# AnteMarusic/Accelerating-Genomics

Hardware: AMD Instinct MI355X
Metric: Smith-Waterman affine-gap score-only GCUPS (config 2: 65536 pairs 150x150 per GPU) (higher is better)
Workload: dtype int16x2 lanes, int32 scores; 1 GPU; BASELINE config 2: 65536 SW pairs 150x150 per GPU, iid ACGT + 25% related, newline sentinel aligned as the reference does; pairs_per_gpu=65536, len=150, cells_counted_per_pair=22500, parallelism=pairs sharded per GPU, no collective

## Files before the change

accelerating-genomics_amd/api.py:

```python
from __future__ import annotations

import ctypes as C
import os
import subprocess

import numpy as np

_HERE = os.path.dirname(os.path.abspath(__file__))
TUNING_KNOBS = ("AGX_SW_KERNEL", "AGX_SW_TAIL_BETA", "AGX_SW_MAX_C", "AGX_SW_FORCE_C", "AGX_SW_MAX_CLASSES", "AGX_SW_WAVES_PER_CLASS",
                "AGX_SW_SORT_WAVES", "AGX_SW_ONE_LAUNCH", "AGX_SW_DNA", "AGX_SW_RISE", "AGX_SW_PERIOD", "AGX_PHMM_PLAIN_CELL", "AGX_TRACE_CREATE", "AGX_HOST_THREADS", "AGX_FANOUT", "AGX_PHMM_TAB_BUDGET", "AGX_PHMM_MAX_C",
                "AGX_PHMM_FORCE_C", "AGX_PHMM_TAIL_BETA", "AGX_PHMM_MAX_CLASSES", "AGX_PHMM_NO_LUT", "AGX_TRACE_POOL", "AGX_NO_STREAM_PRIO", "AGX_SW_I32_CLASSIC", "AGX_SW_PIECE_MB", "AGX_SW_PIECE_MIN_PAIRS", "AGX_PHMM_NO_ROWS", "AGX_PHMM_NO_TRAINS", "AGX_PHMM_LUT_ONE_LOOP", "AGX_SW_HOST_PLAN", "AGX_PHMM_NO_RING", "AGX_TRACE_CIGAR")
_DEFAULT_LIB = "libagx_tuning.so" if any(k in os.environ for k in TUNING_KNOBS) else "libagx.so"
LIB_PATH = os.environ.get("AGX_LIB_PATH", os.path.join(_HERE, _DEFAULT_LIB))

OK, E_ARG, E_NODEVICE, E_HIP, E_NOMEM, E_SYMBOL, E_LIMIT, E_IO, E_INTERNAL = 0, -1, -2, -3, -4, -5, -6, -7, -8
SW_ALIGN_ENDS, SW_ALIGN_SPANS = 1, 2
SW_ALIGN_MAX_QUERY_LEN, SW_ALIGN_MAX_TARGET_LEN = 2560, 65535
SW_MODE_LOCAL, SW_MODE_GLOBAL, SW_MODE_FIT, SW_MODE_EXTEND, SW_MODE_EXTEND_QUERY = 0, 1, 2, 3, 4
SwHit = np.dtype([("score", np.int32), ("a_begin", np.int32), ("a_end", np.int32), ("b_begin", np.int32), ("b_end", np.int32)])
SwStat = np.dtype([("matches", np.int32), ("pairs", np.int32)])
SW_STATS_MAX_QUERY_LEN = 1792
SW_CIGAR_MAX_QUERY_LEN = 2048
SW_BAND_MAX_LEN = 65535
SW_BAND_MAX_WIDTH = 2048
CIGAR_INS, CIGAR_DEL, CIGAR_EQ, CIGAR_DIFF = 1, 2, 7, 8
_CIGAR_CHARS = {CIGAR_INS: "I", CIGAR_DEL: "D", CIGAR_EQ: "=", CIGAR_DIFF: "X"}
OPT_SW_KERNEL = 1
OPT_SW_PLANNER = 2
SW_PLANNER_AUTO, SW_PLANNER_HOST, SW_PLANNER_DEVICE = 0, 1, 2
OPT_PHMM_TRAINS = 3
OPT_SW_TRACE_BYTES = 4
PHMM_TRAINS_AUTO, PHMM_TRAINS_OFF, PHMM_TRAINS_ON = 0, 1, 2
SW_KERNEL_AUTO, SW_KERNEL_INT32, SW_KERNEL_PACKED_SIGNED, SW_KERNEL_PACKED_BIASED = 0, 1, 2, 3
PHMM_F64, PHMM_F64_FMA, PHMM_F32, PHMM_F32_FMA = 0, 1, 2, 3
# ... 663 lines not shown
```

accelerating-genomics_amd/csrc/agx_sw.cpp:

```cpp
#include "agx_sw_batch.h"

#include <cmath>
#include <memory>
#include <mutex>
#include <thread>

#include "agx_parallel.h"

using namespace agx_sw_host;

namespace {

struct Tiling {
    int cls;
    int G;
};

bool positive(long n) { return n > 0; }
bool at_least_4(long n) { return n >= 4; }
inline double tail_beta_override() { static const double v = agx_knob_real(agx_tune("AGX_SW_TAIL_BETA"), -1.0); return v; }
int max_cols_per_lane() { static const int v = (int)agx_knob_int(agx_tune("AGX_SW_MAX_C"), AGX_SW_MAX_COLS_PER_LANE, at_least_4); return v; }
int force_cols_per_lane() { static const int v = (int)agx_knob_int(agx_tune("AGX_SW_FORCE_C"), 0); return v; }
int max_classes_override() { static const int v = (int)agx_knob_int(agx_tune("AGX_SW_MAX_CLASSES"), 0, positive); return v; }
int tuned_kernel()
// ... 121 lines not shown
    return best;
}

inline uint64_t piece_bytes() { static const uint64_t v = (uint64_t)agx_knob_int(agx_tune("AGX_SW_PIECE_MB"), 32, positive) << 20; return v; }
inline int64_t piece_min_pairs() { static const int64_t v = agx_knob_int(agx_tune("AGX_SW_PIECE_MIN_PAIRS"), 32768, positive); return v; }
constexpr size_t kRawPad = 64;
constexpr uint8_t kClsEmpty = 255;
constexpr uint8_t kClsUntiled = 254;
struct PairPlan {
    uint32_t pair;
    uint32_t ly;
    uint16_t lxo;
    uint8_t cls;
    uint8_t G;
    uint32_t lx() const { return lxo & 0x7fffu; }
};

struct Bucket {
    size_t first = 0, count = 0;
    size_t group0 = 0, n_groups = 0;
    size_t wave0 = 0, n_waves = 0;
    int cls = 0, G = 0;
};

}

namespace {
int finish_create(agx_sw_batch *b);
void drop_pending(agx_sw_batch *b);
}

extern "C" {

void agx_sw_batch_destroy(agx_sw_batch *b)
{
    if (!b) return;
    if (b->ctx) (void)hipSetDevice(b->ctx->device);
    drop_pending(b);
    b->img.release();
    b->groups.release();
    b->waves.release();
    b->scores.release();
    b->table.release();
    b->out_stage.release();
    b->ends.release();
    b->ends_stage.release();
// ... 815 lines not shown
    t_sort = agx_now_ms();
    }

    size_t n_groups = 0, n_waves_total = 0, groups_bytes = 0, waves_bytes = 0;
    const size_t img0 = packed ? (size_t)kSwPackedMaxShort / 4 + 1 : 0;
    size_t img_dw = img0;
    std::vector<SwWave> waves;
    std::vector<ClassLaunch> launches;
    uint32_t launched_classes = 0;
    int64_t padded = 0;
    double t_waves = t_sort, t_records = t_sort;
    std::vector<uint8_t> groups_host;
    if (device_plan) {
        {
            static std::mutex once_per_context;
            std::lock_guard<std::mutex> l(once_per_context);
            rc = agx_ctx_prepare_plan(ctx);
        }
        if (!rc) rc = dp.h_buckets.alloc(ctx, (size_t)kSwPlanBuckets * 5 * sizeof(uint32_t));
        if (rc) return rc;
        uint32_t *bt = (uint32_t *)dp.h_buckets.p;
        size_t entries = 0, n_waves = 0;
        uint32_t class_mask = 0;
        for (int k = 0; k < kSwPlanBuckets; ++k) {
            const size_t count = dp.hist[(size_t)k];
            const int G = 64 - (k & 63);
            const size_t ng = (count + slots - 1) / slots, per_wave = (size_t)(64 / G), nw = (ng + per_wave - 1) / per_wave;
            bt[5 * k + 0] = (uint32_t)entries;
            bt[5 * k + 1] = (uint32_t)count;
            bt[5 * k + 2] = (uint32_t)n_groups;
            bt[5 * k + 3] = (uint32_t)ng;
            bt[5 * k + 4] = (uint32_t)n_waves;
            entries += count;
            n_groups += ng;
            n_waves += nw;
            if (count) class_mask |= 1u << (k >> 6);
        }
        n_waves_total = n_waves;
        launched_classes = class_mask;
        img_dw = dp.img_dw;
        groups_bytes = n_groups * sizeof(SwGroup2);
        waves_bytes = n_waves * sizeof(SwWave);
        ClassLaunch cl;
        cl.C = (class_mask & (class_mask - 1)) ? 0 : kSwClasses[__builtin_ctz(class_mask)];
        cl.first_wave = 0;
        cl.n_waves = (uint32_t)n_waves;
        launches.assign(1, cl);
        rc = launch_device_plan(ctx, dp, b, (uint32_t)n_pairs, (uint32_t)entries, longest_long, slots, (uint32_t)img0, n_groups, n_waves);
        if (!rc) rc = h_flag.alloc(ctx, 2 * sizeof(uint32_t));
        if (rc) return rc;
        t_waves = t_records = agx_now_ms();
    } else {
    std::vector<Bucket> bk;
    for (size_t i = 0; i < plan.size();) {
        Bucket q;
        q.first = i;
        q.cls = plan[i].cls;
        q.G = plan[i].G;
        size_t lo = i, hi = plan.size();
        while (lo + 1 < hi) {
            const size_t mid = lo + (hi - lo) / 2;
            if (plan[mid].cls == q.cls && plan[mid].G == q.G) lo = mid;
            else hi = mid;
        }
        q.count = lo + 1 - i;
        i = lo + 1;
        bk.push_back(q);
    }
    size_t n_waves = 0;
// ... 32 lines not shown
        const char *e = agx_tune("AGX_SW_SORT_WAVES");
        return !(e && e[0] == '0');
    }();
    static const bool one_launch_ok = [] {
        const char *e = agx_tune("AGX_SW_ONE_LAUNCH");
        return !(e && e[0] == '0');
    }();
    if (coded_plan && launches.size() > 1 && one_launch_ok) {
        if (sort_waves)
            std::stable_sort(waves.begin(), waves.end(), [](const SwWave &a, const SwWave &b) {
                return (uint64_t)a.steps * a.reserved > (uint64_t)b.steps * b.reserved;
            });
        ClassLaunch all_classes;
        all_classes.C = 0;
        all_classes.first_wave = 0;
        all_classes.n_waves = (uint32_t)waves.size();
        launches.assign(1, all_classes);
    } else if (sort_waves && !launches.empty())
        agx_pool_run((int)launches.size(), [&](int k) {
            const ClassLaunch &cl = launches[(size_t)k];
            std::stable_sort(waves.begin() + cl.first_wave, waves.begin() + cl.first_wave + cl.n_waves,
                             [](const SwWave &a, const SwWave &b) { return a.steps > b.steps; });
        });
    std::vector<uint32_t> x_dw(plan.size()), y_dw(plan.size());
    img_dw = img0;
    {
        const int parts = (int)std::min<int64_t>(agx_host_threads(), std::max<int64_t>(1, (int64_t)plan.size() / 16384));
        std::vector<size_t> part_sum((size_t)parts + 1, 0);
        const size_t chunk = (plan.size() + parts - 1) / (size_t)parts;
        auto words = [&](const PairPlan &pp, size_t *xw) {
            *xw = ((size_t)pp.G * kSwClasses[pp.cls] + 3) / 4 + 1;
            return *xw + ((size_t)pp.ly + 3) / 4;
        };
        agx_pool_run(parts, [&](int t) {
            const size_t lo = std::min(plan.size(), (size_t)t * chunk), hi = std::min(plan.size(), lo + chunk);
            size_t s = 0, xw;
            for (size_t i = lo; i < hi; ++i) s += words(plan[i], &xw);
            part_sum[(size_t)t + 1] = s;
        });
        for (int t = 0; t < parts; ++t) part_sum[(size_t)t + 1] += part_sum[(size_t)t];
        img_dw = img0 + part_sum[(size_t)parts];
        if (img_dw > 0xffffffffull) {
            agx_set_error("packed image exceeds 16 GiB; split the batch");
            return AGX_E_LIMIT;
        }
        agx_pool_run(parts, [&](int t) {
// ... 217 lines not shown
        return AGX_E_NODEVICE;
    }
    int rc = agx_bind(b->ctx);
    if (rc) return rc;
    if (b->banded) return band_launch(b);
    if (b->pending && b->pending->ready) AGX_HIP(hipStreamWaitEvent(b->ctx->stream, b->pending->ready, 0));
    SwParams prm = b->prm;
    if (b->bound) prm.n_out = (uint32_t)b->n_pairs;
    b->cig_valid = false;
    if (b->cigar == 2 && !b->trace_p && b->tr_dwords) {
        agx_set_error("agx_sw_batch_launch: a traced fill without its trace block");
        return AGX_E_INTERNAL;
    }
    FanOut fan(b->ctx, (int)b->launches.size());
    rc = fan.begin();
    if (rc) return rc;
    int k = 0;
    for (auto it = b->launches.rbegin(); it != b->launches.rend(); ++it) {
        const ClassLaunch &cl = *it;
        hipStream_t st = fan.stream(k++);
        const uint32_t *img = (const uint32_t *)b->img.p;
        const SwWave *wv = (const SwWave *)b->waves.p + cl.first_wave;
        int32_t *scores = b->bound ? b->bound : (int32_t *)b->scores.p;
        const int anch_capture = b->mode != AGX_SW_MODE_EXTEND, anch_flags = b->mode == AGX_SW_MODE_FIT ? 1 : b->mode == AGX_SW_MODE_GLOBAL ? 2 : 0;
        int r;
        uint32_t *lstat = (uint32_t *)b->lstat.p;
        if (b->cigar == 2 && b->matrix)
            r = agx_sw_trace_mat_launch_class(cl.C, prm, img, (const SwGroup *)b->groups.p, wv, cl.n_waves, scores, (uint32_t *)b->ends.p, b->trace_p,
                                              (const uint64_t *)b->goff.p, (const int16_t *)b->table.p, st);
        else if (b->cigar == 2)
            r = agx_sw_trace_launch_class(cl.C, prm, img, (const SwGroup *)b->groups.p, wv, cl.n_waves, scores, (uint32_t *)b->ends.p, b->trace_p,
                                          (const uint64_t *)b->goff.p, st);
        else if (b->stats == 2 && b->family == 5 && b->matrix)
            r = agx_sw_anch_mat_stats_launch_class(cl.C, anch_capture, anch_flags, prm, img, (const SwGroup *)b->groups.p, wv, cl.n_waves, scores,
                                                   (uint32_t *)b->ends.p, lstat, (const int16_t *)b->table.p, st);
        else if (b->stats == 2 && b->family == 5)
            r = agx_sw_anch_stats_launch_class(cl.C, anch_capture, anch_flags, prm, img, (const SwGroup *)b->groups.p, wv, cl.n_waves, scores,
                                               (uint32_t *)b->ends.p, lstat, st);
        else if (b->stats == 2 && b->matrix)
            r = agx_sw_loc_mat_stats_launch_class(cl.C, prm, img, (const SwGroup *)b->groups.p, wv, cl.n_waves, scores, (uint32_t *)b->ends.p, lstat,
                                                  (const int16_t *)b->table.p, st);
        else if (b->stats == 2)
            r = agx_sw_loc_stats_launch_class(cl.C, prm, img, (const SwGroup *)b->groups.p, wv, cl.n_waves, scores, (uint32_t *)b->ends.p, lstat, st);
        else if (b->family == 5 && b->matrix)
            r = agx_sw_anch_mat_launch_class(cl.C, anch_capture, anch_flags, prm, img, (const SwGroup *)b->groups.p, wv, cl.n_waves, scores,
                                             (uint32_t *)b->ends.p, (const int16_t *)b->table.p, st);
// ... 210 lines not shown
```

accelerating-genomics_amd/csrc/agx_sw.h:

```cpp
#pragma once
#include <hip/hip_runtime.h>

#include <algorithm>
#include <cstdint>

#include "../../include/agx.h"

struct SwGroup {
    uint32_t x_dw;
    uint32_t y_dw;
    uint32_t lx_ly;
    uint32_t out;
};

struct SwParams {
    int32_t ge;
    int32_t gf;
    int32_t hd;
    int32_t delta;
    int32_t shift;
    uint32_t ge2, gf2, hd2, delta2;
    uint32_t age2, agf2, bias2;
    uint32_t n_out;
};

struct SwGroup2 {
    uint32_t x_dw[2];
    uint32_t y_dw[2];
    uint32_t lx_ly[2];
    uint32_t out[2];
};

struct SwWave {
    uint32_t first_group;
    uint16_t n_groups;
    uint16_t G;
    uint32_t steps;
    uint32_t reserved;
};

#define AGX_SW_FOR_EACH_CLASS(X) \
    X(4) X(6) X(8) X(10) X(12) X(14) X(16) X(18) X(20) X(22) X(24) X(26) X(28) X(30) X(32) X(34) X(36) X(38) X(40)
#define AGX_SW_FOR_EACH_WIDE_CLASS(X) X(80) X(120) X(160)
static const int kSwClasses[] = {4, 6, 8, 10, 12, 14, 16, 18, 20, 22, 24, 26, 28, 30, 32, 34, 36, 38, 40, 80, 120, 160};
static const int kSwPackedMaxShort = 64 * 40;
static const int kSwNumClasses = sizeof(kSwClasses) / sizeof(kSwClasses[0]);
static const double kSwClassCost[] = {1.373, 1.250, 1.178, 1.138, 1.112, 1.080, 1.051, 1.033, 1.025, 1.022, 1.014, 1.014, 1.011, 1.007, 1.007, 1.004, 1.004, 1.004, 1.000, 1.6, 2.2, 4.0};
static const double kSwPkClassCost[] = {1.543, 1.358, 1.278, 1.210, 1.173, 1.136, 1.111, 1.086, 1.068, 1.037, 1.025, 1.025, 1.019, 1.012, 1.006, 1.006, 1.006, 1.000, 1.000, 0, 0, 0};
static const double kSwPk2ClassCost[] = {1.851, 1.581, 1.450, 1.367, 1.318, 1.263, 1.196, 1.184, 1.145, 1.097, 1.095, 1.056, 1.049, 1.053, 1.025, 1.023, 1.022, 1.016, 1.000, 0, 0, 0};

static const double kSwI32dClassCost[] = {1.373, 1.250, 1.178, 1.138, 1.112, 1.080, 1.051, 1.033, 1.025, 1.022, 1.014, 1.014, 1.011, 1.007, 1.007, 1.004, 1.004, 1.004, 1.000, 0, 0, 0};

constexpr int kSwMatDim = 33;
int agx_sw_mat_launch_class(int cols_per_lane, const SwParams &prm, const uint32_t *img, const SwGroup *groups,
                            const SwWave *waves, uint32_t n_waves, int32_t *scores, const int16_t *table, hipStream_t s);
int agx_sw_pack_launch(bool matrix, int slots, const uint8_t *raw, const uint64_t *off, uint64_t base, const void *groups,
                       uint32_t n_groups, uint32_t n_pairs, uint32_t *img, const uint8_t *code, uint32_t *flag, int n_cu,
                       hipStream_t s);
int agx_sw_pack_dna_launch(const uint8_t *raw, const uint64_t *off, uint64_t base, void *groups, void *waves, uint32_t n_waves,
                           uint32_t n_pairs, uint32_t *img, uint32_t *flag, int n_cu, hipStream_t s);
int agx_sw_pk_launch_class(int cols_per_lane, const SwParams &prm, const uint32_t *img, const SwGroup2 *groups,
                           const SwWave *waves, uint32_t n_waves, int32_t *scores, hipStream_t s);
// ... 147 lines not shown
```

accelerating-genomics_amd/csrc/agx_sw_batch.h:

```cpp
#pragma once
#include "agx_sw.h"

#include <algorithm>

#include "agx_internal.h"

namespace agx_sw_host __attribute__((visibility("hidden"))) {

struct ClassLaunch {
    int C = 0;
    uint32_t first_wave = 0, n_waves = 0;
};

}

struct agx_sw_batch {
    agx_ctx *ctx = nullptr;
    int family = 0;
    int align = 0;
    int mode = 0;
    int stats = 0;
    DevBuf lstat;
    PinBuf lstat_stage;
    int cigar = 0;
    std::vector<uint64_t> tr_goff;
    std::vector<SwWalkRec> tr_walk;
    uint64_t tr_dwords = 0, tr_slot_words = 0;
    DevBuf goff, walkrec;
    uint32_t *trace_p = nullptr;
    bool cig_valid = false;
    std::vector<agx_sw_hit> cig_hits;
    std::vector<uint64_t> cig_off;
    std::vector<uint32_t> cig_ops;
    agx_sw_cigar_info cig_info{};
// ... 87 lines not shown
```

accelerating-genomics_amd/csrc/agx_sw_pack_kernel.hip:

```cpp
#include "agx_sw.h"

namespace {

template <bool MAT>
__device__ __forceinline__ uint32_t fetch(const uint8_t *__restrict__ seq, uint32_t idx, uint32_t len,
                                          const uint8_t *__restrict__ code, bool &bad)
{
    if (idx >= len) return 0u;
    uint32_t b = seq[idx];
    if constexpr (MAT) {
        const uint32_t c = code[b];
        bad |= c == 0xffu;
        b = (c + 1u) & 0xffu;
    } else
        bad |= b == 0u;
    return b;
}

template <bool MAT>
__device__ __forceinline__ void copy_seq(uint32_t *__restrict__ dst, uint32_t n_dw, const uint8_t *__restrict__ seq, uint32_t len,
                                         const uint8_t *__restrict__ code, int lane, bool &bad)
{
    for (uint32_t i = lane; i < n_dw; i += 64) {
        uint32_t v = 0;
// ... 75 lines not shown

__device__ __forceinline__ uint32_t find_entry(const uint32_t *s_pre, uint32_t c)
{
    uint32_t lo = 0;
#pragma unroll
    for (uint32_t step = kPackEntries / 2; step; step >>= 1)
        if (s_pre[lo + step] <= c) lo += step;
    return lo;
}

__global__ void __launch_bounds__(256) sw_pack_dna(const uint8_t *__restrict__ raw, const uint64_t *__restrict__ off, uint64_t base,
                                                   uint32_t *__restrict__ groups, uint32_t *__restrict__ waves, uint32_t n_fill_waves,
                                                   uint32_t n_pairs, uint32_t *__restrict__ img, uint32_t *__restrict__ flag)
{
    __shared__ uint32_t s_bits[128][8];
    __shared__ uint64_t s_src[kPackEntries];
    __shared__ uint32_t s_len[kPackEntries];
    __shared__ uint32_t s_flags[kPackEntries];
    __shared__ uint32_t s_pre[kPackEntries + 1];
    __shared__ uint32_t s_wsum[4];
    __shared__ uint32_t s_info[128], s_syms[128];
    __shared__ uint32_t s_dst[kPackEntries], s_wlen[kPackEntries];
    __shared__ uint32_t s_not_dna;
    const uint32_t e = threadIdx.x, sl = e >> 1, which = e & 1u;
    for (uint32_t i = threadIdx.x; i < 128 * 8; i += 256) (&s_bits[0][0])[i] = 0;
    for (uint32_t fw = blockIdx.x; fw < n_fill_waves; fw += gridDim.x) {
        const uint32_t first_group = waves[4 * (size_t)fw], n_groups = waves[4 * (size_t)fw + 1] & 0xffffu;
        const uint32_t gc = (waves[4 * (size_t)fw + 1] >> 16) * (waves[4 * (size_t)fw + 3] & 0xffffu);
        const uint32_t n_slots = n_groups * 2u;
        if (threadIdx.x == 0) s_not_dna = 0;
        uint32_t *rec = groups + (size_t)(first_group + (sl >> 1)) * 8u;
        const uint32_t h = sl & 1u;
        uint32_t len = 0, nl = 0, x_dw = 0, y_dw = 0, lx = 0, ly = 0, xsec = 0, out = n_pairs;
        uint64_t src = 0;
        if (sl < n_slots) {
            x_dw = rec[h], y_dw = rec[2 + h];
            const uint32_t ll = rec[4 + h];
            out = rec[6 + h];
            if (out < n_pairs) {
                lx = ll & 0x7fffu, xsec = (ll >> 15) & 1u, ly = ll >> 16;
                src = off[2 * (size_t)out + (which ? xsec ^ 1u : xsec)] - base;
                len = which ? ly : lx;
                nl = len && raw[src + len - 1] == '\n';
            }
        }
        s_src[e] = src;
        s_len[e] = len - nl;
        s_flags[e] = 0;
        {
            const uint32_t span = (uint32_t)(src & 15u) + (len - nl);
            block_scan256(len - nl ? (span + 15u) >> 4 : 0u, s_pre, s_wsum);
        }
        const uint32_t total1 = s_pre[kPackEntries];
// ... 111 lines not shown
                    }
                    o[w] = v;
                }
            } else {
#pragma unroll
                for (uint32_t w = 0; w < 4; ++w) {
                    uint32_t v = 0;
#pragma unroll
                    for (uint32_t j = 0; j < 4; ++j) {
                        const int32_t idx = first + (int32_t)(4 * w + j);
                        if (idx >= 0 && idx < (int32_t)n) v |= q.w[w] & (0xffu << (8 * j));
                    }
                    o[w] = v;
                }
            }
            uint32_t *d = img + s_dst[ce] + 4u * k;
#pragma unroll
            for (uint32_t w = 0; w < 4; ++w)
                if (4u * k + w < nw) d[w] = o[w];
        }
        if (all_dna) {
            if (which == 0 && sl < n_slots && out < n_pairs) {
                const uint32_t info = s_info[sl], xnl = (info >> 4) & 1u, ynl = (info >> 5) & 1u;
                rec[4 + h] = (lx - xnl) | ((xnl & ynl) << 13) | (xsec << 15) | ((ly - ynl) << 16);
            }
            if (threadIdx.x == 0) waves[4 * (size_t)fw + 3] |= 1u << 16;
        }
        __syncthreads();
    }
}

}

int agx_sw_pack_dna_launch(const uint8_t *raw, const uint64_t *off, uint64_t base, void *groups, void *waves, uint32_t n_waves,
                           uint32_t n_pairs, uint32_t *img, uint32_t *flag, int n_cu, hipStream_t s)
{
    if (n_waves == 0) return 0;
    static_assert(sizeof(SwWave) == 16 && sizeof(SwGroup2) == 32, "sw_pack_dna reads the records as words");
    const uint32_t blocks = (uint32_t)std::min<uint64_t>((uint64_t)n_waves, (uint64_t)std::max(n_cu, 1) * 32u);
    hipLaunchKernelGGL(sw_pack_dna, dim3(blocks), dim3(256), 0, s, raw, off, base, (uint32_t *)groups, (uint32_t *)waves, n_waves, n_pairs,
                       img, flag);
    return hipGetLastError() == hipSuccess ? 0 : -1;
}

int agx_sw_pack_launch(bool matrix, int slots, const uint8_t *raw, const uint64_t *off, uint64_t base, const void *groups,
                       uint32_t n_groups, uint32_t n_pairs, uint32_t *img, const uint8_t *code, uint32_t *flag, int n_cu,
                       hipStream_t s)
{
    if (n_groups == 0) return 0;
    const uint64_t total = (uint64_t)n_groups * (uint64_t)slots;
    const uint32_t blocks = (uint32_t)std::min<uint64_t>((total + 3) / 4, (uint64_t)std::max(n_cu, 1) * 16u);
// ... 16 lines not shown
```

accelerating-genomics_amd/csrc/agx_sw_pk2_kernel.hip:

```cpp
#include "agx_sw_pk2_kernel.inc"

namespace {

template <int C, int KC>
__global__ void __launch_bounds__(256) sw_fill_pk2(const SwParams prm, const uint32_t *__restrict__ img,
                                                   const SwGroup2 *__restrict__ groups,
                                                   const SwWave *__restrict__ waves, uint32_t n_waves,
                                                   int32_t *__restrict__ scores)
{
    const uint32_t wave = __builtin_amdgcn_readfirstlane(blockIdx.x * 4u + (threadIdx.x >> 6));
    if (wave >= n_waves) return;
    pk2_body<C, KC>(prm, img, groups, waves[wave], scores);
}

template <int KC>
__global__ void __launch_bounds__(256) sw_fill_pk2_any(const SwParams prm, const uint32_t *__restrict__ img,
                                                       const SwGroup2 *__restrict__ groups,
                                                       const SwWave *__restrict__ waves, uint32_t n_waves,
                                                       int32_t *__restrict__ scores)
{
    const uint32_t wave = __builtin_amdgcn_readfirstlane(blockIdx.x * 4u + (threadIdx.x >> 6));
    if (wave >= n_waves) return;
    const SwWave w = waves[wave];
    switch (__builtin_amdgcn_readfirstlane(w.reserved) & 0xffffu) {
#define AGX_SW_CASE(CC) \
    case CC: pk2_body<CC, KC>(prm, img, groups, w, scores); break;
        AGX_SW_FOR_EACH_CLASS(AGX_SW_CASE)
#undef AGX_SW_CASE
    default: break;
    }
}

template <int C, int KC>
int launch(const SwParams &prm, const uint32_t *img, const SwGroup2 *groups, const SwWave *waves, uint32_t n_waves,
           int32_t *scores, hipStream_t s)
{
    const uint32_t blocks = (n_waves + 3) / 4;
    hipLaunchKernelGGL((sw_fill_pk2<C, KC>), dim3(blocks), dim3(256), 0, s, prm, img, groups, waves, n_waves, scores);
    return hipGetLastError() == hipSuccess ? 0 : -1;
}

}

int agx_sw_pk2_launch_any(int rising, bool wide, const SwParams &prm, const uint32_t *img, const SwGroup2 *groups, const SwWave *waves,
                          uint32_t n_waves, int32_t *scores, hipStream_t s)
{
    if (n_waves == 0) return 0;
    if (rising == 4 && wide) return agx_sw_pk2w_launch_any(prm, img, groups, waves, n_waves, scores, s);
    const uint32_t blocks = (n_waves + 3) / 4;
// ... 30 lines not shown
```

accelerating-genomics_amd/csrc/agx_sw_pk2_kernel.inc:

```
#include "agx_sw.h"
#include <type_traits>

namespace {

typedef unsigned short u16x2 __attribute__((ext_vector_type(2)));

__device__ __forceinline__ u16x2 as_v(uint32_t v) { return __builtin_bit_cast(u16x2, v); }
__device__ __forceinline__ uint32_t as_u(u16x2 v) { return __builtin_bit_cast(uint32_t, v); }
__device__ __forceinline__ uint32_t umax2(uint32_t a, uint32_t b) { return as_u(__builtin_elementwise_max(as_v(a), as_v(b))); }
__device__ __forceinline__ uint32_t umin2(uint32_t a, uint32_t b) { return as_u(__builtin_elementwise_min(as_v(a), as_v(b))); }
typedef _Float16 f16x2 __attribute__((ext_vector_type(2)));
__device__ __forceinline__ uint32_t umax3(uint32_t a, uint32_t b, uint32_t c)
{
    const f16x2 x = __builtin_bit_cast(f16x2, a), y = __builtin_bit_cast(f16x2, b), z = __builtin_bit_cast(f16x2, c);
    return __builtin_bit_cast(uint32_t, __builtin_elementwise_maximum(__builtin_elementwise_maximum(x, y), z));
}
__device__ __forceinline__ uint32_t in_vgpr(uint32_t s)
{
    uint32_t r;
    asm volatile("v_mov_b32 %0, %1" : "=v"(r) : "s"(s));
    return r;
}

#define AGX_DPP_TAKE " wave_shr:1 row_mask:0xf bank_mask:0xf bound_ctrl:0\n"
// ... 62 lines not shown
    constexpr int NF = FQ ? NM : NK;
    uint32_t floorv[NF];
#pragma unroll
    for (int k = 0; k < NF; ++k) floorv[k] = (RISE ? bias + prm.age2 : bias) + (uint32_t)k * prm.age2;
    const uint32_t z_init = RISE ? z0 + prm.age2 : z0;
    const uint32_t kv = in_vgpr((prm.delta2 & 0xffu) << 24);
    const uint64_t start_mask = __ballot(start);
    const uint32_t lx_mask = FAST ? 0xfffu : 0x7fffu;
    const int lxA = (int)(g.lx_ly[0] & lx_mask), lxB = (int)(g.lx_ly[1] & lx_mask);
    const int lyA = (int)(g.lx_ly[0] >> 16), lyB = (int)(g.lx_ly[1] >> 16);

    const uint32_t no_row = FAST ? 0x1f1f1f1fu : 0u;
    const uint32_t *ybA = lyA > 0 ? img + g.y_dw[0] : img, *ybB = lyB > 0 ? img + g.y_dw[1] : img;
    const uint32_t lastA = lyA > 0 ? (uint32_t)((lyA + 3) >> 2) - 1u : 0u, lastB = lyB > 0 ? (uint32_t)((lyB + 3) >> 2) - 1u : 0u;
    const int nqA = feeder ? (lyA + 3) >> 2 : 0, nqB = feeder ? (lyB + 3) >> 2 : 0;
    auto loadA = [&](int q) -> uint32_t { return ybA[min((uint32_t)q, lastA)]; };
    auto loadB = [&](int q) -> uint32_t { return ybB[min((uint32_t)q, lastB)]; };
    auto row_selA = [&](int q, uint32_t v) -> uint32_t { return q < nqA ? v : no_row; };
    auto row_selB = [&](int q, uint32_t v) -> uint32_t { return q < nqB ? v : no_row; };

    uint32_t xq[C];
    constexpr int PF = C < 8 ? 2 : 1;
    uint32_t nextA[PF], nextB[PF];
    {
        const uint32_t o = (uint32_t)gl * C, d0 = o >> 2, sh = o & 3u;
        const uint32_t fillA = (FAST && !(active && g.x_dw[0])) ? 0x0c0c0c0cu : 0u;
        const uint32_t fillB = (FAST && !(active && g.x_dw[1])) ? 0x0c0c0c0cu : 0u;
        uint32_t ra[XW + 1], rb[XW + 1];
#pragma unroll
        for (int k = 0; k <= XW; ++k) {
            ra[k] = img[g.x_dw[0] + d0 + k];
            rb[k] = img[g.x_dw[1] + d0 + k];
        }
#pragma unroll
        for (int r = 0; r < PF; ++r) {
            nextA[r] = loadA(r);
            nextB[r] = loadB(r);
        }
        __builtin_amdgcn_s_waitcnt(0x0f70);
        __builtin_amdgcn_sched_barrier(0);
#pragma unroll
        for (int k = 0; k <= XW; ++k) {
            ra[k] |= fillA;
            rb[k] |= fillB;
        }
#pragma unroll
        for (int k = 0; k < XW; ++k) {
            const uint32_t a = __builtin_amdgcn_alignbyte(ra[k + 1], ra[k], sh);
            const uint32_t b = __builtin_amdgcn_alignbyte(rb[k + 1], rb[k], sh);
#pragma unroll
            for (int i = 0; i < 4; ++i)
                if (4 * k + i < C) {
                    const uint32_t ca = (a >> (8 * i)) & 0xffu, cb = (b >> (8 * i)) & 0xffu;
                    uint32_t v;
                    if constexpr (FAST)
                        v = ca | 0x0c00u | (cb << 16) | 0x0c000000u;
                    else {
                        const int col = (int)o + 4 * k + i;
                        v = (col < lxA ? ca << sh_sym : col_pad) | ((col < lxB ? cb << sh_sym : col_pad) << 16);
                    }
                    asm volatile("" : "+v"(v));
                    xq[4 * k + i] = v;
                }
        }
    }

    uint32_t z[C], e[C];
#pragma unroll
    for (int j = 0; j < C; ++j) {
        z[j] = z_init + (uint32_t)(j % NK) * prm.age2;
        e[j] = bias + (uint32_t)(j % NK) * prm.age2;
    }
    uint32_t z_last = z_init + (uint32_t)kEnd * prm.age2, f_last = z_last, diag_in = z0 + (uint32_t)kEnd * prm.age2;
    uint32_t best[NM];
#pragma unroll
    for (int k = 0; k < NM; ++k) best[k] = z_init + (uint32_t)(KC > 1 ? k + 1 : k) * prm.age2;
    uint32_t yc = 0;
    uint32_t ta = 0, tb = 0;

    const bool last = active && gl == G - 1;
    const bool nlA = FAST && last && ((g.lx_ly[0] >> 13) & 1u), nlB = FAST && last && ((g.lx_ly[1] >> 13) & 1u);
    const int capA_t = (nlA && lxA > 0 && lyA > 0) ? lyA + G - 2 : -1, capB_t = (nlB && lxB > 0 && lyB > 0) ? lyB + G - 2 : -1;
    uint32_t cornerA = z_init + (uint32_t)kEnd * prm.age2, cornerB = cornerA;

    const int steps = (int)w.steps;
    uint32_t rowsA = 0, rowsB = 0;
    int t = 0;

    auto take_max = [&](auto sc) __attribute__((always_inline)) {
        constexpr int S = decltype(sc)::value;
#pragma unroll
        for (int k = 0; k < NK; ++k) {
#pragma unroll
            for (int j = k; j < C; j += 2 * NK) {
                if (j + NK < C)
                    best[S + k] = umax3(best[S + k], z[j], z[j + NK]);
                else
                    best[S + k] = umax2(best[S + k], z[j]);
            }
// ... 70 lines not shown
#pragma unroll
            for (int m = 0; m < NM; ++m) best[m] += ge4;
        }
        if constexpr (FQ) {
#pragma unroll
            for (int m = 0; m < NF; ++m) floorv[m] += 4u * prm.age2;
        }
    };
    auto quad_of_steps = [&](auto cc) __attribute__((always_inline)) {
        step(std::integral_constant<int, 0>{}, std::integral_constant<int, 0>{}, cc);
        step(std::integral_constant<int, 1>{}, std::integral_constant<int, 1>{}, cc);
        step(std::integral_constant<int, 2>{}, std::integral_constant<int, 2>{}, cc);
        step(std::integral_constant<int, 3>{}, std::integral_constant<int, 3>{}, cc);
        rise4();
    };
    auto take = [&](int q, int r) __attribute__((always_inline)) {
        rowsA = row_selA(q, nextA[r]);
        rowsB = row_selB(q, nextB[r]);
        nextA[r] = loadA(q + PF);
        nextB[r] = loadB(q + PF);
        if constexpr (WIDE) __builtin_amdgcn_sched_barrier(0);
    };
    const int quads = steps >> 2;
    int cap_first = 0x7fffffff;
    if constexpr (FAST) {
        cap_first = min(capA_t < 0 ? 0x7fffffff : capA_t, capB_t < 0 ? 0x7fffffff : capB_t);
        for (int o = 32; o > 0; o >>= 1) cap_first = min(cap_first, __shfl_xor(cap_first, o));
        cap_first = __builtin_amdgcn_readfirstlane(cap_first);
    }
    const int quads_free = min(quads, cap_first >> 2);
    constexpr std::integral_constant<bool, false> no_cap{};
    constexpr std::integral_constant<bool, FAST> cap{};
    int q = 0;
    if constexpr (PF == 1) {
        if constexpr (FAST) {
            for (; q < quads_free; ++q) {
                take(q, 0);
                quad_of_steps(no_cap);
            }
        }
        for (; q < quads; ++q) {
            take(q, 0);
            quad_of_steps(cap);
        }
    } else {
        if constexpr (FAST) {
            for (; q + 1 < quads_free; q += 2) {
                take(q, 0);
                quad_of_steps(no_cap);
                take(q + 1, 1);
                quad_of_steps(no_cap);
            }
        }
// ... 42 lines not shown
        best[0] = umax2(best[0], cand);
    }
    uint32_t bestv = best[0];
    for (int o = 1; o < G; o <<= 1) {
        const uint32_t other = (uint32_t)__shfl_down((int)bestv, o);
        if (gl + o < G) bestv = umax2(bestv, other);
    }
    {
        const int off = (int)(z0 & 0xffffu) + (RISE ? (steps + 1) * (int)(prm.age2 & 0xffffu) : 0);
        const int src = (lane * G) & 63;
        const int sa = __shfl((int)(bestv & 0xffffu) - off, src), sb = __shfl((int)(bestv >> 16) - off, src);
        const uint32_t oa = (uint32_t)__shfl((int)g.out[0], src), ob = (uint32_t)__shfl((int)g.out[1], src);
        if (lane < (int)w.n_groups) {
            if (ob == oa + 1u && !(oa & 1u) && ob < prm.n_out)
                *reinterpret_cast<int2 *>(scores + oa) = make_int2(sa, sb);
            else {
                scores[oa] = sa;
                if (ob < prm.n_out) scores[ob] = sb;
            }
        }
    }
}

template <int C, int KC, bool WIDE = false>
__device__ __forceinline__ void pk2_body(const SwParams &prm, const uint32_t *__restrict__ img, const SwGroup2 *__restrict__ groups,
                                         const SwWave w, int32_t *__restrict__ scores)
{
    static_assert(C % 2 == 0, "the running maximum takes two columns per instruction");
    constexpr int KCC = KC > 1 && C < 14 ? 1 : KC;
    constexpr bool W = WIDE && KCC > 1 && sw_pk2_period(C) > 4;
    const int lane = threadIdx.x & 63;
    const int G = w.G;
    const int grp = lane / G;
    const int gl = lane - grp * G;
    const bool active = grp < (int)w.n_groups;
    const bool start = gl == 0;
    const bool feeder = active && start;

    SwGroup2 g = groups[w.first_group + (active ? grp : 0)];
    __builtin_amdgcn_s_waitcnt(0x0f70);
    __builtin_amdgcn_sched_barrier(0);
#pragma unroll
    for (int k = 0; k < 2; ++k) {
        g.x_dw[k] = active ? g.x_dw[k] : 0u;
        g.y_dw[k] = active ? g.y_dw[k] : 0u;
        g.lx_ly[k] = active ? g.lx_ly[k] : 0u;
        g.out[k] = active ? g.out[k] : 0u;
    }
    if (__builtin_amdgcn_readfirstlane(w.reserved >> 16) & 1u)
        pk2_fill<C, true, KCC, W>(prm, img, g, w, scores, lane, G, gl, active, start, feeder);
    else
        pk2_fill<C, false, KCC, W>(prm, img, g, w, scores, lane, G, gl, active, start, feeder);
}

}
```

accelerating-genomics_amd/csrc/agx_sw_pk2w_kernel.hip:

```cpp
#include "agx_sw_pk2_kernel.inc"

namespace {

template <int C>
__global__ void __launch_bounds__(256) sw_fill_pk2w(const SwParams prm, const uint32_t *__restrict__ img,
                                                    const SwGroup2 *__restrict__ groups,
                                                    const SwWave *__restrict__ waves, uint32_t n_waves,
                                                    int32_t *__restrict__ scores)
{
    const uint32_t wave = __builtin_amdgcn_readfirstlane(blockIdx.x * 4u + (threadIdx.x >> 6));
    if (wave >= n_waves) return;
    pk2_body<C, 4, true>(prm, img, groups, waves[wave], scores);
}

__global__ void __launch_bounds__(256) sw_fill_pk2w_any(const SwParams prm, const uint32_t *__restrict__ img,
                                                        const SwGroup2 *__restrict__ groups,
                                                        const SwWave *__restrict__ waves, uint32_t n_waves,
                                                        int32_t *__restrict__ scores)
{
    const uint32_t wave = __builtin_amdgcn_readfirstlane(blockIdx.x * 4u + (threadIdx.x >> 6));
    if (wave >= n_waves) return;
    const SwWave w = waves[wave];
    switch (__builtin_amdgcn_readfirstlane(w.reserved) & 0xffffu) {
#define AGX_SW_CASE(CC) \
    case CC: pk2_body<CC, 4, true>(prm, img, groups, w, scores); break;
        AGX_SW_FOR_EACH_CLASS(AGX_SW_CASE)
#undef AGX_SW_CASE
    default: break;
    }
}

template <int C>
int launch(const SwParams &prm, const uint32_t *img, const SwGroup2 *groups, const SwWave *waves, uint32_t n_waves,
           int32_t *scores, hipStream_t s)
{
    if constexpr (sw_pk2_period(C) > 4) {
        const uint32_t blocks = (n_waves + 3) / 4;
        hipLaunchKernelGGL((sw_fill_pk2w<C>), dim3(blocks), dim3(256), 0, s, prm, img, groups, waves, n_waves, scores);
        return hipGetLastError() == hipSuccess ? 0 : -1;
    } else
        return -2;
}

}

int agx_sw_pk2w_launch_any(const SwParams &prm, const uint32_t *img, const SwGroup2 *groups, const SwWave *waves, uint32_t n_waves,
                           int32_t *scores, hipStream_t s)
{
// ... 25 lines not shown
```

Baseline: 9148 GCUPS.

## Speculatively load group records in kernel head and precompute corner cap in pack

Before the wave descriptor arrives, the kernel head guesses each lane's group-record address from a host-supplied base, stride and G, so the record load and the descriptor load are in flight together. If the guess is wrong it falls back to an inline-asm reload. The pack kernel now computes the first corner step per fill wave and stores it in the wave's reserved field, which replaces the in-kernel cross-lane shuffle reduction. The z/e/best initialisation is moved ahead of the waitcnt so it overlaps the prefetch loads, at the cost of more head complexity and possible register pressure.

```diff
diff --git a/accelerating-genomics_amd/api.py b/accelerating-genomics_amd/api.py
--- a/accelerating-genomics_amd/api.py
+++ b/accelerating-genomics_amd/api.py
@@ -9,7 +9,7 @@
 _HERE = os.path.dirname(os.path.abspath(__file__))
 TUNING_KNOBS = ("AGX_SW_KERNEL", "AGX_SW_TAIL_BETA", "AGX_SW_MAX_C", "AGX_SW_FORCE_C", "AGX_SW_MAX_CLASSES", "AGX_SW_WAVES_PER_CLASS",
                 "AGX_SW_SORT_WAVES", "AGX_SW_ONE_LAUNCH", "AGX_SW_DNA", "AGX_SW_RISE", "AGX_SW_PERIOD", "AGX_PHMM_PLAIN_CELL", "AGX_TRACE_CREATE", "AGX_HOST_THREADS", "AGX_FANOUT", "AGX_PHMM_TAB_BUDGET", "AGX_PHMM_MAX_C",
-                "AGX_PHMM_FORCE_C", "AGX_PHMM_TAIL_BETA", "AGX_PHMM_MAX_CLASSES", "AGX_PHMM_NO_LUT", "AGX_TRACE_POOL", "AGX_NO_STREAM_PRIO", "AGX_SW_I32_CLASSIC", "AGX_SW_PIECE_MB", "AGX_SW_PIECE_MIN_PAIRS", "AGX_PHMM_NO_ROWS", "AGX_PHMM_NO_TRAINS", "AGX_PHMM_LUT_ONE_LOOP", "AGX_SW_HOST_PLAN", "AGX_PHMM_NO_RING", "AGX_TRACE_CIGAR")
+                "AGX_PHMM_FORCE_C", "AGX_PHMM_TAIL_BETA", "AGX_PHMM_MAX_CLASSES", "AGX_PHMM_NO_LUT", "AGX_TRACE_POOL", "AGX_NO_STREAM_PRIO", "AGX_SW_I32_CLASSIC", "AGX_SW_PIECE_MB", "AGX_SW_PIECE_MIN_PAIRS", "AGX_PHMM_NO_ROWS", "AGX_PHMM_NO_TRAINS", "AGX_PHMM_LUT_ONE_LOOP", "AGX_SW_HOST_PLAN", "AGX_PHMM_NO_RING", "AGX_TRACE_CIGAR", "AGX_SW_HEAD_GUESS")
 _DEFAULT_LIB = "libagx_tuning.so" if any(k in os.environ for k in TUNING_KNOBS) else "libagx.so"
 LIB_PATH = os.environ.get("AGX_LIB_PATH", os.path.join(_HERE, _DEFAULT_LIB))
 
diff --git a/accelerating-genomics_amd/csrc/agx_sw.cpp b/accelerating-genomics_amd/csrc/agx_sw.cpp
--- a/accelerating-genomics_amd/csrc/agx_sw.cpp
+++ b/accelerating-genomics_amd/csrc/agx_sw.cpp
@@ -167,6 +167,17 @@
     size_t wave0 = 0, n_waves = 0;
     int cls = 0, G = 0;
 };
+
+void head_guess(agx_sw_host::ClassLaunch &cl, const SwWave *waves)
+{
+    if (!cl.n_waves) return;
+    const SwWave *w = waves + cl.first_wave;
+    uint32_t count = w[0].n_groups;
+    for (uint32_t k = 1; k + 1 < cl.n_waves && count; ++k)
+        if (w[k].n_groups != count) count = 0;
+    cl.g_base = w[0].first_group;
+    cl.g_count = count | (uint32_t)w[0].G << 16;
+}
 
 }
 
@@ -1028,9 +1039,11 @@
         uint32_t *bt = (uint32_t *)dp.h_buckets.p;
         size_t entries = 0, n_waves = 0;
         uint32_t class_mask = 0;
+        int filled = 0, filled_G = 1;
         for (int k = 0; k < kSwPlanBuckets; ++k) {
             const size_t count = dp.hist[(size_t)k];
             const int G = 64 - (k & 63);
+            if (count) ++filled, filled_G = G;
             const size_t ng = (count + slots - 1) / slots, per_wave = (size_t)(64 / G), nw = (ng + per_wave - 1) / per_wave;
             bt[5 * k + 0] = (uint32_t)entries;
             bt[5 * k + 1] = (uint32_t)count;
@@ -1051,6 +1064,7 @@
         cl.C = (class_mask & (class_mask - 1)) ? 0 : kSwClasses[__builtin_ctz(class_mask)];
         cl.first_wave = 0;
         cl.n_waves = (uint32_t)n_waves;
+        if (filled == 1) cl.g_count = (uint32_t)(64 / filled_G) | (uint32_t)filled_G << 16;
         launches.assign(1, cl);
         rc = launch_device_plan(ctx, dp, b, (uint32_t)n_pairs, (uint32_t)entries, longest_long, slots, (uint32_t)img0, n_groups, n_waves);
         if (!rc) rc = h_flag.alloc(ctx, 2 * sizeof(uint32_t));
@@ -1129,6 +1143,7 @@
             std::stable_sort(waves.begin() + cl.first_wave, waves.begin() + cl.first_wave + cl.n_waves,
                              [](const SwWave &a, const SwWave &b) { return a.steps > b.steps; });
         });
+    for (ClassLaunch &cl : launches) head_guess(cl, waves.data());
     std::vector<uint32_t> x_dw(plan.size()), y_dw(plan.size());
     img_dw = img0;
     {
@@ -1392,6 +1407,13 @@
         const uint32_t *img = (const uint32_t *)b->img.p;
         const SwWave *wv = (const SwWave *)b->waves.p + cl.first_wave;
         int32_t *scores = b->bound ? b->bound : (int32_t *)b->scores.p;
+        if (b->family == 2) {
+            prm.g_base = cl.g_base;
+            prm.g_count = cl.g_count;
+            prm.g_last = (uint32_t)(b->groups.bytes / sizeof(SwGroup2)) - 1u;
+            if (const char *e = agx_tune("AGX_SW_HEAD_GUESS"))
+                if (e[0] == 'w') prm.g_base = cl.g_base + 1u + cl.n_waves * 64u;
+        }
         const int anch_capture = b->mode != AGX_SW_MODE_EXTEND, anch_flags = b->mode == AGX_SW_MODE_FIT ? 1 : b->mode == AGX_SW_MODE_GLOBAL ? 2 : 0;
         int r;
         uint32_t *lstat = (uint32_t *)b->lstat.p;
diff --git a/accelerating-genomics_amd/csrc/agx_sw.h b/accelerating-genomics_amd/csrc/agx_sw.h
--- a/accelerating-genomics_amd/csrc/agx_sw.h
+++ b/accelerating-genomics_amd/csrc/agx_sw.h
@@ -22,6 +22,7 @@
     uint32_t ge2, gf2, hd2, delta2;
     uint32_t age2, agf2, bias2;
     uint32_t n_out;
+    uint32_t g_base, g_count, g_last;
 };
 
 struct SwGroup2 {
@@ -38,6 +39,19 @@
     uint32_t steps;
     uint32_t reserved;
 };
+
+constexpr int kSwCornerShift = 17;
+constexpr uint32_t kSwCornerNone = 0x7fffu;
+constexpr uint32_t kSwNoCornerStep = 0xffffffffu;
+__host__ __device__ inline uint32_t sw_corner_step(uint32_t ll, uint32_t G)
+{
+    const uint32_t lx = ll & 0xfffu, ly = ll >> 16;
+    return ((ll >> 13) & 1u) && lx && ly ? ly + G - 2u : kSwNoCornerStep;
+}
+__host__ __device__ inline uint32_t sw_corner_field(uint32_t first_step)
+{
+    return first_step == kSwNoCornerStep ? kSwCornerNone : first_step >> 2;
+}
 
 #define AGX_SW_FOR_EACH_CLASS(X) \
     X(4) X(6) X(8) X(10) X(12) X(14) X(16) X(18) X(20) X(22) X(24) X(26) X(28) X(30) X(32) X(34) X(36) X(38) X(40)
diff --git a/accelerating-genomics_amd/csrc/agx_sw_batch.h b/accelerating-genomics_amd/csrc/agx_sw_batch.h
--- a/accelerating-genomics_amd/csrc/agx_sw_batch.h
+++ b/accelerating-genomics_amd/csrc/agx_sw_batch.h
@@ -10,6 +10,7 @@
 struct ClassLaunch {
     int C = 0;
     uint32_t first_wave = 0, n_waves = 0;
+    uint32_t g_base = 0, g_count = 1u << 16;
 };
 
 }
diff --git a/accelerating-genomics_amd/csrc/agx_sw_pack_kernel.hip b/accelerating-genomics_amd/csrc/agx_sw_pack_kernel.hip
--- a/accelerating-genomics_amd/csrc/agx_sw_pack_kernel.hip
+++ b/accelerating-genomics_amd/csrc/agx_sw_pack_kernel.hip
@@ -121,13 +121,15 @@
     __shared__ uint32_t s_info[128], s_syms[128];
     __shared__ uint32_t s_dst[kPackEntries], s_wlen[kPackEntries];
     __shared__ uint32_t s_not_dna;
+    __shared__ uint32_t s_corner;
     const uint32_t e = threadIdx.x, sl = e >> 1, which = e & 1u;
     for (uint32_t i = threadIdx.x; i < 128 * 8; i += 256) (&s_bits[0][0])[i] = 0;
     for (uint32_t fw = blockIdx.x; fw < n_fill_waves; fw += gridDim.x) {
         const uint32_t first_group = waves[4 * (size_t)fw], n_groups = waves[4 * (size_t)fw + 1] & 0xffffu;
         const uint32_t gc = (waves[4 * (size_t)fw + 1] >> 16) * (waves[4 * (size_t)fw + 3] & 0xffffu);
+        const uint32_t lanes_per_group = waves[4 * (size_t)fw + 1] >> 16;
         const uint32_t n_slots = n_groups * 2u;
-        if (threadIdx.x == 0) s_not_dna = 0;
+        if (threadIdx.x == 0) s_not_dna = 0, s_corner = kSwNoCornerStep;
         uint32_t *rec = groups + (size_t)(first_group + (sl >> 1)) * 8u;
         const uint32_t h = sl & 1u;
         uint32_t len = 0, nl = 0, x_dw = 0, y_dw = 0, lx = 0, ly = 0, xsec = 0, out = n_pairs;
@@ -285,11 +287,14 @@
         if (all_dna) {
             if (which == 0 && sl < n_slots && out < n_pairs) {
                 const uint32_t info = s_info[sl], xnl = (info >> 4) & 1u, ynl = (info >> 5) & 1u;
-                rec[4 + h] = (lx - xnl) | ((xnl & ynl) << 13) | (xsec << 15) | ((ly - ynl) << 16);
-            }
-            if (threadIdx.x == 0) waves[4 * (size_t)fw + 3] |= 1u << 16;
+                const uint32_t ll = (lx - xnl) | ((xnl & ynl) << 13) | (xsec << 15) | ((ly - ynl) << 16);
+                rec[4 + h] = ll;
+                const uint32_t cs = sw_corner_step(ll, lanes_per_group);
+                if (cs != kSwNoCornerStep) atomicMin(&s_corner, cs);
+            }
         }
         __syncthreads();
+        if (all_dna && threadIdx.x == 0) waves[4 * (size_t)fw + 3] |= (1u << 16) | (sw_corner_field(s_corner) << kSwCornerShift);
     }
 }
 
diff --git a/accelerating-genomics_amd/csrc/agx_sw_pk2_kernel.hip b/accelerating-genomics_amd/csrc/agx_sw_pk2_kernel.hip
--- a/accelerating-genomics_amd/csrc/agx_sw_pk2_kernel.hip
+++ b/accelerating-genomics_amd/csrc/agx_sw_pk2_kernel.hip
@@ -8,9 +8,10 @@
                                                    const SwWave *__restrict__ waves, uint32_t n_waves,
                                                    int32_t *__restrict__ scores)
 {
-    const uint32_t wave = __builtin_amdgcn_readfirstlane(blockIdx.x * 4u + (threadIdx.x >> 6));
-    if (wave >= n_waves) return;
-    pk2_body<C, KC>(prm, img, groups, waves[wave], scores);
+    SwWave w;
+    SwLanes l;
+    if (!pk2_head(prm, n_waves, groups, waves, img, scores, w, l)) return;
+    pk2_body<C, KC>(prm, img, w, l, scores);
 }
 
 template <int KC>
@@ -19,12 +20,12 @@
                                                        const SwWave *__restrict__ waves, uint32_t n_waves,
                                                        int32_t *__restrict__ scores)
 {
-    const uint32_t wave = __builtin_amdgcn_readfirstlane(blockIdx.x * 4u + (threadIdx.x >> 6));
-    if (wave >= n_waves) return;
-    const SwWave w = waves[wave];
+    SwWave w;
+    SwLanes l;
+    if (!pk2_head(prm, n_waves, groups, waves, img, scores, w, l)) return;
     switch (__builtin_amdgcn_readfirstlane(w.reserved) & 0xffffu) {
 #define AGX_SW_CASE(CC) \
-    case CC: pk2_body<CC, KC>(prm, img, groups, w, scores); break;
+    case CC: pk2_body<CC, KC>(prm, img, w, l, scores); break;
         AGX_SW_FOR_EACH_CLASS(AGX_SW_CASE)
 #undef AGX_SW_CASE
     default: break;
diff --git a/accelerating-genomics_amd/csrc/agx_sw_pk2_kernel.inc b/accelerating-genomics_amd/csrc/agx_sw_pk2_kernel.inc
--- a/accelerating-genomics_amd/csrc/agx_sw_pk2_kernel.inc
+++ b/accelerating-genomics_amd/csrc/agx_sw_pk2_kernel.inc
@@ -108,6 +108,8 @@
     uint32_t xq[C];
     constexpr int PF = C < 8 ? 2 : 1;
     uint32_t nextA[PF], nextB[PF];
+    uint32_t z[C], e[C];
+    uint32_t best[NM];
     {
         const uint32_t o = (uint32_t)gl * C, d0 = o >> 2, sh = o & 3u;
         const uint32_t fillA = (FAST && !(active && g.x_dw[0])) ? 0x0c0c0c0cu : 0u;
@@ -122,6 +124,18 @@
         for (int r = 0; r < PF; ++r) {
             nextA[r] = loadA(r);
             nextB[r] = loadB(r);
+        }
+        __builtin_amdgcn_sched_barrier(0);
+#pragma unroll
+        for (int j = 0; j < C; ++j) {
+            z[j] = z_init + (uint32_t)(j % NK) * prm.age2;
+            e[j] = bias + (uint32_t)(j % NK) * prm.age2;
+            if constexpr (WIDE) asm volatile("" : "+v"(e[j]));
+        }
+#pragma unroll
+        for (int k = 0; k < NM; ++k) {
+            best[k] = z_init + (uint32_t)(KC > 1 ? k + 1 : k) * prm.age2;
+            if constexpr (WIDE) asm volatile("" : "+v"(best[k]));
         }
         __builtin_amdgcn_s_waitcnt(0x0f70);
         __builtin_amdgcn_sched_barrier(0);
@@ -151,16 +165,7 @@
         }
     }
 
-    uint32_t z[C], e[C];
-#pragma unroll
-    for (int j = 0; j < C; ++j) {
-        z[j] = z_init + (uint32_t)(j % NK) * prm.age2;
-        e[j] = bias + (uint32_t)(j % NK) * prm.age2;
-    }
     uint32_t z_last = z_init + (uint32_t)kEnd * prm.age2, f_last = z_last, diag_in = z0 + (uint32_t)kEnd * prm.age2;
-    uint32_t best[NM];
-#pragma unroll
-    for (int k = 0; k < NM; ++k) best[k] = z_init + (uint32_t)(KC > 1 ? k + 1 : k) * prm.age2;
     uint32_t yc = 0;
     uint32_t ta = 0, tb = 0;
 
@@ -277,13 +282,7 @@
         if constexpr (WIDE) __builtin_amdgcn_sched_barrier(0);
     };
     const int quads = steps >> 2;
-    int cap_first = 0x7fffffff;
-    if constexpr (FAST) {
-        cap_first = min(capA_t < 0 ? 0x7fffffff : capA_t, capB_t < 0 ? 0x7fffffff : capB_t);
-        for (int o = 32; o > 0; o >>= 1) cap_first = min(cap_first, __shfl_xor(cap_first, o));
-        cap_first = __builtin_amdgcn_readfirstlane(cap_first);
-    }
-    const int quads_free = min(quads, cap_first >> 2);
+    const int quads_free = FAST ? min(quads, (int)(__builtin_amdgcn_readfirstlane(w.reserved) >> kSwCornerShift)) : quads;
     constexpr std::integral_constant<bool, false> no_cap{};
     constexpr std::integral_constant<bool, FAST> cap{};
     int q = 0;
@@ -372,24 +371,70 @@
     }
 }
 
+typedef uint32_t u32x4 __attribute__((ext_vector_type(4)));
+struct SwLanes {
+    int G, grp;
+    u32x4 lo, hi;
+};
+static_assert(sizeof(SwGroup2) == 32 && sizeof(SwWave) == 16, "pk2_head loads the records as 16-byte words");
+
+__device__ __forceinline__ bool pk2_head(const SwParams &prm, uint32_t n_waves, const SwGroup2 *__restrict__ groups,
+                                         const SwWave *__restrict__ waves, const void *img, const void *scores, SwWave &w, SwLanes &l)
+{
+    const uint32_t wave = __builtin_amdgcn_readfirstlane(blockIdx.x * 4u + (threadIdx.x >> 6));
+    uint32_t nw = n_waves;
+    asm("" : "+s"(nw) : "s"(groups), "s"(waves), "s"(img), "s"(scores), "s"(prm.g_base), "s"(prm.g_count), "s"(prm.g_last), "s"(prm.hd2),
+        "s"(prm.delta2), "s"(prm.age2), "s"(prm.agf2), "s"(prm.bias2), "s"(prm.n_out));
+    if (wave >= nw) return false;
+    const int lane = threadIdx.x & 63;
+    const uint32_t first = prm.g_base + wave * (prm.g_count & 0xffffu);
+    int G = (int)(prm.g_count >> 16);
+    int grp = lane / G;
+    u32x4 wr = *reinterpret_cast<const u32x4 *>(waves + wave);
+    const u32x4 *rec = reinterpret_cast<const u32x4 *>(groups + min(first + (uint32_t)grp, prm.g_last));
+    u32x4 lo = rec[0], hi = rec[1];
+    asm volatile("" : "+s"(wr));
+    w.first_group = wr.x;
+    w.n_groups = (uint16_t)(wr.y & 0xffffu);
+    w.G = (uint16_t)(wr.y >> 16);
+    w.steps = wr.z;
+    w.reserved = wr.w;
+    if (w.first_group != first || (int)w.G != G) {
+        G = w.G;
+        grp = lane / G;
+        rec = reinterpret_cast<const u32x4 *>(groups + min(w.first_group + (uint32_t)grp, prm.g_last));
+        asm volatile("global_load_dwordx4 %0, %2, off\n"
+                     "global_load_dwordx4 %1, %2, off offset:16\n"
+                     "s_waitcnt vmcnt(0)"
+                     : "+v"(lo), "+v"(hi)
+                     : "v"(rec)
+                     : "memory");
+    }
+    l.G = G;
+    l.grp = grp;
+    l.lo = lo;
+    l.hi = hi;
+    return true;
+}
+
 template <int C, int KC, bool WIDE = false>
-__device__ __forceinline__ void pk2_body(const SwParams &prm, const uint32_t *__restrict__ img, const SwGroup2 *__restrict__ groups,
-                                         const SwWave w, int32_t *__restrict__ scores)
+__device__ __forceinline__ void pk2_body(const SwParams &prm, const uint32_t *__restrict__ img, const SwWave w, const SwLanes l,
+                                         int32_t *__restrict__ scores)
 {
     static_assert(C % 2 == 0, "the running maximum takes two columns per instruction");
     constexpr int KCC = KC > 1 && C < 14 ? 1 : KC;
     constexpr bool W = WIDE && KCC > 1 && sw_pk2_period(C) > 4;
     const int lane = threadIdx.x & 63;
-    const int G = w.G;
-    const int grp = lane / G;
+    const int G = l.G;
+    const int grp = l.grp;
     const int gl = lane - grp * G;
     const bool active = grp < (int)w.n_groups;
     const bool start = gl == 0;
     const bool feeder = active && start;
 
-    SwGroup2 g = groups[w.first_group + (active ? grp : 0)];
     __builtin_amdgcn_s_waitcnt(0x0f70);
     __builtin_amdgcn_sched_barrier(0);
+    SwGroup2 g = {{l.lo.x, l.lo.y}, {l.lo.z, l.lo.w}, {l.hi.x, l.hi.y}, {l.hi.z, l.hi.w}};
 #pragma unroll
     for (int k = 0; k < 2; ++k) {
         g.x_dw[k] = active ? g.x_dw[k] : 0u;
diff --git a/accelerating-genomics_amd/csrc/agx_sw_pk2w_kernel.hip b/accelerating-genomics_amd/csrc/agx_sw_pk2w_kernel.hip
--- a/accelerating-genomics_amd/csrc/agx_sw_pk2w_kernel.hip
+++ b/accelerating-genomics_amd/csrc/agx_sw_pk2w_kernel.hip
@@ -8,9 +8,10 @@
                                                     const SwWave *__restrict__ waves, uint32_t n_waves,
                                                     int32_t *__restrict__ scores)
 {
-    const uint32_t wave = __builtin_amdgcn_readfirstlane(blockIdx.x * 4u + (threadIdx.x >> 6));
-    if (wave >= n_waves) return;
-    pk2_body<C, 4, true>(prm, img, groups, waves[wave], scores);
+    SwWave w;
+    SwLanes l;
+    if (!pk2_head(prm, n_waves, groups, waves, img, scores, w, l)) return;
+    pk2_body<C, 4, true>(prm, img, w, l, scores);
 }
 
 __global__ void __launch_bounds__(256) sw_fill_pk2w_any(const SwParams prm, const uint32_t *__restrict__ img,
@@ -18,12 +19,12 @@
                                                         const SwWave *__restrict__ waves, uint32_t n_waves,
                                                         int32_t *__restrict__ scores)
 {
-    const uint32_t wave = __builtin_amdgcn_readfirstlane(blockIdx.x * 4u + (threadIdx.x >> 6));
-    if (wave >= n_waves) return;
-    const SwWave w = waves[wave];
+    SwWave w;
+    SwLanes l;
+    if (!pk2_head(prm, n_waves, groups, waves, img, scores, w, l)) return;
     switch (__builtin_amdgcn_readfirstlane(w.reserved) & 0xffffu) {
 #define AGX_SW_CASE(CC) \
-    case CC: pk2_body<CC, 4, true>(prm, img, groups, w, scores); break;
+    case CC: pk2_body<CC, 4, true>(prm, img, w, l, scores); break;
         AGX_SW_FOR_EACH_CLASS(AGX_SW_CASE)
 #undef AGX_SW_CASE
     default: break;
```

Result: no change. 9191 GCUPS, median of 3 (+0.5%).
